# VITA-Group/CV_A-FAN

Measured on AMD Instinct MI355X. Metric: images/sec (whole node) A-FAN K=5 train step, ResNet-18/CIFAR-10, higher is better.
Workload: dtype bf16; 1 GPU; resnet18 CIFAR-10-shape A-FAN K=5 bf16, batch 256/GPU, perturb_idx 6, internal layout nhwc, 1xMI355X per rank (BASELINE configs[1]); global_batch=256, parallelism=dp1, hipgraph=True, in_launch_batchnorm=True

## Files before the change

### cv_a-fan_amd/_lib.py

```python
import ctypes as C
import os

_HERE = os.path.dirname(os.path.abspath(__file__))
LIB_PATH = os.environ.get("AFAN_HIP_LIB") or os.path.join(_HERE, "libafan_hip.so")

AFAN_F32, AFAN_BF16 = 0, 1
AFAN_NCHW, AFAN_NHWC = 0, 1
AFAN_ESHAPE = -3
_ERRORS = {-1: "AFAN_EDTYPE (unknown dtype code)", -2: "AFAN_EALIGN (misaligned pointer)",
           AFAN_ESHAPE: "AFAN_ESHAPE (bad sizes)", -4: "AFAN_ENULL (required pointer is NULL)",
           -5: "AFAN_ELAYOUT (unknown layout code)"}

_p, _i, _l, _f = C.c_void_p, C.c_int, C.c_int64, C.c_float

SIGNATURES = {
    "afan_version": (_i, []),
    "afan_arch": (C.c_char_p, []),
    "afan_pgd_step": (_i, [_p, _p, _i, _p, _p, _l, _f, _f, _i, _p]),
    "afan_tensor_clamp": (_i, [_p, _p, _p, _l, _p]),
    "afan_norms_workspace_floats": (_l, [_l, _l]),
    "afan_pgd_step_norms": (_i, [_p, _p, _i, _p, _p, _l, _l, _f, _f, _i, _p, _p, _p, _p]),
    "afan_perturb_norms": (_i, [_p, _p, _l, _l, _p, _p, _p, _p]),
    "afan_pgd_step_l2_workspace_floats": (_l, [_l, _l]),
    "afan_pgd_step_l2": (_i, [_p, _p, _i, _p, _p, _l, _l, _f, _f, _i, _p, _p, _p, _p]),
    "afan_axpy_noise": (_i, [_p, _p, _l, _f, _p, _p]),
    "afan_pgd_rand_start": (_i, [_p, _p, _p, _l, _l, _l, _l, _i, _f, _p, _p, _i, _p]),
    "afan_mix_feature": (_i, [_p, _p, _p, _l, _l, _l, _f, _i, _p]),
    "afan_mix_feature_nhwc": (_i, [_p, _p, _p, _l, _l, _l, _f, _i, _p]),
    "afan_lerp_points": (_i, [_p, _p, _p, _l, C.POINTER(_f), _i, _p]),
    "afan_lerp_mix": (_i, [_p, _p, _p, _l, _l, _l, C.POINTER(_f), _i, C.c_uint, _f, _i, _p]),
    "afan_sat_points_nhwc": (_i, [_p, _p, _p, _i, _l, _l, C.POINTER(_f), _i, C.c_uint, _f, _p]),
    "afan_head_max_classes": (_i, []),
    "afan_head_forward": (_i, [_p, _i, _l, _l, _l, _p, _p, _l, _p, _p, _p]),
    "afan_head_backward": (_i, [_p, _p, _p, _l, _l, _l, _l, _p, _i, _p, _p, _i, _p]),
    "afan_cross_entropy": (_i, [_p, _p, _l, _l, _p, _p, _p]),
    "afan_head_ce": (_i, [_p, _p, _i, _l, _l, _l, _p, _p, _p, _l, _p, _f, _p, _p, _p, _p, _p, _p, _p]),
    "afan_loss_mean": (_i, [_p, _l, _p, _p]),
    "afan_mix_w_workspace_floats": (_l, []),
    "afan_mix_w": (_i, [_p, _p, _p, _p, _i, _l, _p]),
    "afan_mix_w_backward": (_i, [_p, _i, _p, _p, _l, _p, _p, _i, _p]),
    "afan_bn_workspace_floats": (_l, [_l]),
    "afan_bn_acc_doubles": (_l, [_l]),
    "afan_bn_acc_supported": (_i, [_i, _l]),
    "afan_bn_set_running_updates": (_i, [_i]),
    "afan_bn_running_update": (_i, [_p, _l, C.c_double, _f, _f, _p, _p, _p, _p]),
    "afan_bn_running_update_batched": (_i, [_p, _p, _p, _p, _p, _p, _p, _p, _i, _p]),
    "afan_bn_train_forward_acc": (_i, [_p, _p, _p, _i, _l, _l, _l, _f, _f, _p, _p, _i, _p, _i, _p, _p, _p, _p, _i, _p]),
    "afan_bn_train_forward_acc_dual": (_i, [_p, _p, _p, _i, _l, _l, _l, _f, _f, _p, _p, _p, _p, _p, _p, _p, _f, _f, _p, _p, _p, _p,
                                            _p, _p, _p, _p]),
    "afan_bn_backward_acc": (_i, [_p, _p, _p, _p, _p, _i, _l, _l, _l, _p, _i, _p, _i, _p, _p, _i, _i, _p]),
    "afan_bn_backward_rows": (_i, [_p, _p, _p, _p, _p, _i, _l, _l, _l, _p, _p, _p, _p, _i, _p]),
    "afan_bn_backward_acc_rows": (_i, [_p, _p, _p, _p, _p, _i, _l, _l, _l, _p, _p, _p, _p, _i, _p]),
    "afan_bn_stats": (_i, [_p, _i, _i, _l, _l, _l, _f, _f, _p, _p, _p, _p, _p, _p]),
    "afan_bn_train_forward": (_i, [_p, _p, _p, _i, _i, _l, _l, _l, _f, _f, _p, _p, _i, _p, _p, _p, _p, _p, _p]),
    "afan_bn_apply": (_i, [_p, _p, _p, _i, _i, _l, _l, _l, _p, _p, _p, _p, _i, _p, _p]),
    "afan_bn_backward": (_i, [_p, _p, _p, _p, _p, _i, _i, _l, _l, _l, _p, _p, _p, _i, _p, _p, _p, _i, _p, _l, _p]),
    "afan_conv_supported": (_i, [_l, _l, _i, _i]),
    "afan_conv_fwd_nhwc_bf16": (_i, [_p, _p, _p, _l, _l, _l, _l, _l, _i, _i, _i, _p, _p, _p, _i, _p]),
    "afan_conv_fwd_affine_nhwc_bf16": (_i, [_p, _p, _p, _l, _l, _l, _l, _l, _i, _i, _i, _p, _p, _i, _i, _p]),
    "afan_conv_fwd_multi_nhwc_bf16": (_i, [_p, _p, _p, _i, _l, _l, _l, _l, _l, _p, _i, _p, _p, _p, _i, _p]),
    "afan_conv_fwd_tiles": (_l, [_l, _l, _l, _l, _l, _i, _i]),
    "afan_bn_train_forward_partials": (_i, [_p, _p, _p, _i, _l, _l, _l, _f, _f, _p, _p, _i, _p, _l, _p, _p, _p, _p, _p, _p]),
    "afan_conv_dgrad_nhwc_bf16": (_i, [_p, _p, _p, _l, _l, _l, _l, _l, _i, _i, _i, _p, _p, _p, _i, _p, _p, _p, _i, _p]),
    "afan_conv_dgrad_affine_nhwc_bf16": (_i, [_p, _p, _p, _l, _l, _l, _l, _l, _i, _i, _i, _p, _p, _i, _p]),
    "afan_conv_dgrad_dual_nhwc_bf16": (_i, [_p, _p, _p, _p, _l, _l, _l, _l, _l, _i, _i, _p, _p, _p, _p]),
    "afan_conv_dgrad_sc_nhwc_bf16": (_i, [_p, _p, _p, _p, _l, _l, _l, _l, _l, _p, _p, _i, _p, _p, _p, _p]),
    "afan_grid_barrier_bytes": (_i, []),
    "afan_grid_barrier_error_word": (_i, []),
    "afan_grid_barrier_shared_gpu": (_i, [_i]),
    "afan_conv_fwd_bn_nhwc_bf16": (_i, [_p, _p, _p, _p, _l, _l, _l, _l, _l, _i, _i, _p, _p, _p, _p, _f, _f, _p, _p, _p, _p, _p, _i, _p, _p, _p, _p,
                                        _f, _f, _p, _p, _p, _p, _p, _p]),
    "afan_conv_dgrad_bn_nhwc_bf16": (_i, [_p, _p, _p, _p, _l, _l, _l, _l, _l, _i, _i, _p, _p, _p, _i, _p, _p, _p, _p, _i, _p, _p, _p, _p, _p, _p,
                                          _p, _p]),
    "afan_conv_fwd_multi_bn_nhwc_bf16": (_i, [_p, _p, _p, _i, _l, _l, _l, _l, _l, _p, _i, _p, _p, _p, _p, _p, _p, _f, _f, _p, _p, _p, _p, _i, _p,
                                              _p]),
# ... 129 lines not shown
```

### cv_a-fan_amd/attack_algo.py

```python
import torch

from . import ops, pgd
from .resnet_s import _dense, _like_layout, fused_criterion, tail_end_kwargs

__all__ = ["PGD", "tensor_clamp", "linfball_proj", "l2ball_proj", "mix_feature", "get_sample_points", "last_norms"]

_last = {"l2": None, "linf": None}


def last_norms():
    return _last["l2"], _last["linf"]


def tensor_clamp(t, min, max, in_place=True):
    res = t if in_place else t.clone()
    ops.tensor_clamp_(res.data, min.contiguous(), max.contiguous())
    return res


def linfball_proj(center, radius, t, in_place=True):
    res = t if in_place else t.clone()
    zero = torch.zeros_like(res.data)
    ops.pgd_step_(res.data, zero, 0.0, x_clean=center.contiguous(), eps=float(radius), clip=True)
    return res


def l2ball_proj(center, radius, t, in_place=True):
    res = t if in_place else t.clone()
    data = res.data
    if _dense(data) is not data or data.dtype != torch.float32:
        raise ValueError("l2ball_proj: t must be a dense fp32 tensor (contiguous NCHW or channels_last)")
    ops.pgd_step_l2_(data, None, 0.0, x_clean=_like_layout(center.detach().float(), data), eps=float(radius), clip=True)
    return res


def PGD(x, loss_fn, y=None, model=None, steps=3, gamma=None, start_idx=1, layer_number=16, eps=(2 / 255),
        randinit=False, clip=False, with_norms=False, grad0=None, norm="linf", tail_end=False):
    if x.device.type != "cuda":
        raise ops.AfanLibraryError("PGD: x must live on the MI355X (no CPU path in this build)")
    pgd._check_norm(norm)
    lp = getattr(model, "compute_dtype", torch.float32) == torch.bfloat16
    if grad0 is not None and (randinit or steps < 1):
        raise ValueError("grad0 is the gradient at x: not with randinit, and only when there is a first step")
    x, x_adv, shadow = ops.pgd_init(_dense(x.detach()), want_shadow=lp and grad0 is None and not randinit)
    if lp and shadow is None:
        shadow = torch.empty_like(x, dtype=torch.bfloat16)
    if randinit and norm == "l2":
        u = _like_layout(torch.randn(x_adv.shape).to(x.device, non_blocking=True), x_adv)
        ops.pgd_step_l2_(x_adv, u, eps, clip=False, shadow=shadow)
    elif randinit:
        ops.axpy_noise_(x_adv, torch.rand(x_adv.shape).to(x.device, non_blocking=True), eps, shadow)
    l2 = linf = None
    loss_fn = fused_criterion(loss_fn, model)
    ce_kw = tail_end_kwargs(model, loss_fn, y, ops.one(x.device), want_value=False) if tail_end else {}
    for t in range(steps):
        if t == 0 and grad0 is not None:
            grad = grad0
        else:
            xin = (shadow if lp else x_adv).detach().requires_grad_(True)
            grad = pgd.input_gradient(lambda t: loss_fn(model(t, end_point=layer_number, start_point=start_idx, **ce_kw), y), xin)
        if with_norms and t == steps - 1:
            l2, linf = pgd.step(x_adv, grad, gamma, x, eps, clip, shadow, norms=True, norm=norm)
        else:
            pgd.step(x_adv, grad, gamma, x, eps, clip, shadow, norm=norm)
    if with_norms:
        if l2 is None:
            l2, linf = ops.perturb_norms(x_adv, x)
        _last["l2"], _last["linf"] = l2, linf
    x_adv.requires_grad_(True)
    if lp:
        x_adv._afan_shadow = shadow
    return x_adv


def mix_feature(clean_feature, adv_feature):
    return ops.mix_feature(_dense(clean_feature), _dense(adv_feature), 1e-5)


def sample_points_mixed(pointx, pointy, number, mix):
    px, py = _dense(pointx), _dense(pointy)
    if py.stride() != px.stride():
        py = _like_layout(py, px)
    return [pointx] + ops.lerp_mix(px, py, number, [bool(f) for f in mix])


def get_sample_points(pointx, pointy, number):
    px, py = _dense(pointx), _dense(pointy)
    if py.stride() != px.stride():
        py = _like_layout(py, px)
    inner = ops.lerp_points(px, py, number)
    return [pointx] + inner + [pointy]
```

### cv_a-fan_amd/ops.py

```python
import contextlib
import ctypes as C
import os
import threading

import torch

from . import _lib
from ._lib import AFAN_BF16, AFAN_ESHAPE, AFAN_F32, AFAN_NCHW, AFAN_NHWC, AfanLibraryError, check

_DT = {torch.float32: AFAN_F32, torch.bfloat16: AFAN_BF16}
_ws_cache = {}
_tls = threading.local()
class _Calls(dict):

    def __init__(self, conv, other):
        super().__init__(conv)
        self.other = dict(other)

    def __getitem__(self, k):
        return self.other[k] if k in self.other else super().__getitem__(k)

    def __contains__(self, k):
        return k in self.other or super().__contains__(k)

    def get(self, k, default=None):
        return self[k] if k in self else default

    def __setitem__(self, k, v):
        if k in self.other:
            self.other[k] = v
        else:
            super().__setitem__(k, v)


CALLS = _Calls({"conv_fwd": 0, "conv_dgrad": 0, "conv_wgrad": 0, "conv_general": 0, "vendor_conv": 0, "conv_bn_fused": 0},
               {"batch_crop_flip": 0, "seg_batch_aug": 0, "seg_batch_aug_jitter": 0, "seg_confusion": 0, "det_batch_resize": 0,
                "frozen_stem_image_grad": 0, "sat_points": 0, "head_ce": 0})


def _need(t, name, dtype=None):
    if not isinstance(t, torch.Tensor):
        raise TypeError(f"{name}: expected a torch.Tensor")
    if t.device.type != "cuda":
        raise AfanLibraryError(f"{name}: tensor is on '{t.device}'. The A-FAN kernels are MI355X-only; "
                               "there is no CPU path (the CPU restatement under oracle/ is test infrastructure).")
    if not _dense(t):
        raise ValueError(f"{name}: tensor must be dense (contiguous NCHW or channels_last)")
    if dtype is not None and t.dtype != dtype:
        raise TypeError(f"{name}: expected {dtype}, got {t.dtype}")
    return t


def _dense(t):
    return t.is_contiguous() or (t.dim() == 4 and t.is_contiguous(memory_format=torch.channels_last))


def layout_of(t):
    if t.dim() == 4 and not t.is_contiguous() and t.is_contiguous(memory_format=torch.channels_last):
        return AFAN_NHWC
    return AFAN_NCHW


def _strides_eq(a, b):
    return all(sa == sb for sa, sb, n in zip(a.stride(), b.stride(), a.shape) if n > 1)


def _same_layout(ref, *others):
    for o in others:
        if o is not None and ref.numel() > 0 and (o.shape != ref.shape or not _strides_eq(o, ref)):
            raise ValueError("operands must share shape and memory layout (strides): "
                             f"{tuple(ref.shape)}/{ref.stride()} vs {tuple(o.shape)}/{o.stride()}")


def _ptr(t):
    return None if t is None else C.c_void_p(t.data_ptr())


_raw_stream = torch._C._cuda_getCurrentRawStream


def _stream(t):
    return C.c_void_p(_raw_stream(t.device.index))


def _workspace(ref, nfloats, tag):
    key = (ref.device.index, _raw_stream(ref.device.index), tag)
    ws = _ws_cache.get(key)
    if ws is None or ws.numel() < nfloats:
        ws = torch.empty(max(int(nfloats), 1024), dtype=torch.float32, device=ref.device)
        _ws_cache[key] = ws
# ... 146 lines not shown
        return False


def pgd_step_(x_adv, grad, gamma, x_clean=None, eps=0.0, clip=False, shadow=None):
    lib = _lib.load()
    _need(x_adv, "x_adv", torch.float32)
    _need(grad, "grad")
    if grad.dtype not in _DT or grad.numel() != x_adv.numel():
        raise TypeError("grad must be fp32/bf16 with x_adv's number of elements")
    if clip:
        _need(x_clean, "x_clean", torch.float32)
        if x_clean.numel() != x_adv.numel():
            raise ValueError("x_clean must match x_adv")
    if shadow is not None:
        _need(shadow, "shadow", torch.bfloat16)
    _same_layout(x_adv, grad, x_clean if clip else None, shadow)
    check(lib.afan_pgd_step(_ptr(x_adv), _ptr(grad), _DT[grad.dtype], _ptr(x_clean) if clip else None,
                            _ptr(shadow), x_adv.numel(), float(gamma), float(eps), int(bool(clip)),
                            _stream(x_adv)), "afan_pgd_step")
    return x_adv


def tensor_clamp_(t, lo, hi):
    lib = _lib.load()
    _need(t, "t", torch.float32)
    _need(lo, "min", torch.float32)
    _need(hi, "max", torch.float32)
    if lo.numel() != t.numel() or hi.numel() != t.numel():
        raise ValueError("min/max must match t")
    check(lib.afan_tensor_clamp(_ptr(t), _ptr(lo), _ptr(hi), t.numel(), _stream(t)), "afan_tensor_clamp")
    return t


def pgd_step_norms_(x_adv, grad, gamma, x_clean, eps=0.0, clip=False, shadow=None):
    lib = _lib.load()
    _need(x_adv, "x_adv", torch.float32)
    _need(grad, "grad")
    _need(x_clean, "x_clean", torch.float32)
    if grad.dtype not in _DT or grad.numel() != x_adv.numel() or x_clean.numel() != x_adv.numel():
        raise TypeError("grad/x_clean must match x_adv")
    if shadow is not None:
        _need(shadow, "shadow", torch.bfloat16)
    _same_layout(x_adv, grad, x_clean, shadow)
    batch = x_adv.shape[0]
    per = x_adv.numel() // max(batch, 1)
    out = torch.empty(2, batch, dtype=torch.float32, device=x_adv.device)
    if batch == 0:
        return out[0], out[1]
    ws = _workspace(x_adv, lib.afan_norms_workspace_floats(batch, per), "norms")
    check(lib.afan_pgd_step_norms(_ptr(x_adv), _ptr(grad), _DT[grad.dtype], _ptr(x_clean), _ptr(shadow),
                                  batch, per, float(gamma), float(eps), int(bool(clip)), _ptr(ws),
                                  _ptr(out[0]), _ptr(out[1]), _stream(x_adv)), "afan_pgd_step_norms")
    return out[0], out[1]


def perturb_norms(x_adv, x_clean):
    lib = _lib.load()
    _need(x_adv, "x_adv", torch.float32)
    _need(x_clean, "x_clean", torch.float32)
    if x_clean.numel() != x_adv.numel():
        raise ValueError("x_clean must match x_adv")
    _same_layout(x_adv, x_clean)
    batch = x_adv.shape[0]
    per = x_adv.numel() // max(batch, 1)
    out = torch.empty(2, batch, dtype=torch.float32, device=x_adv.device)
    if batch == 0:
        return out[0], out[1]
    ws = _workspace(x_adv, lib.afan_norms_workspace_floats(batch, per), "norms")
    check(lib.afan_perturb_norms(_ptr(x_adv), _ptr(x_clean), batch, per, _ptr(ws), _ptr(out[0]),
                                 _ptr(out[1]), _stream(x_adv)), "afan_perturb_norms")
    return out[0], out[1]


def pgd_step_l2_(x_adv, grad, gamma, x_clean=None, eps=0.0, clip=False, shadow=None, want_norms=False):
    lib = _lib.load()
    _need(x_adv, "x_adv", torch.float32)
    if grad is not None:
        _need(grad, "grad")
        if grad.dtype not in _DT or grad.numel() != x_adv.numel():
            raise TypeError("grad must be fp32/bf16 with x_adv's number of elements")
    if clip or want_norms:
        _need(x_clean, "x_clean", torch.float32)
        if x_clean.numel() != x_adv.numel():
            raise ValueError("x_clean must match x_adv")
    else:
        x_clean = None
    if shadow is not None:
        _need(shadow, "shadow", torch.bfloat16)
    if x_adv.dim() < 1:
        raise ValueError("x_adv must have a batch dimension")
    _same_layout(x_adv, grad, x_clean, shadow)
    batch = x_adv.shape[0]
    per = x_adv.numel() // max(batch, 1)
    out = torch.empty(2, batch, dtype=torch.float32, device=x_adv.device) if want_norms else None
    if x_adv.numel():
        ws = _workspace(x_adv, lib.afan_pgd_step_l2_workspace_floats(batch, per), "l2_step")
        check(lib.afan_pgd_step_l2(_ptr(x_adv), _ptr(grad), _DT[grad.dtype] if grad is not None else 0, _ptr(x_clean), _ptr(shadow),
                                   batch, per, float(gamma), float(eps), int(bool(clip)), _ptr(ws),
                                   _ptr(out[0]) if want_norms else None, _ptr(out[1]) if want_norms else None, _stream(x_adv)),
              "afan_pgd_step_l2")
    return (x_adv, out[0], out[1]) if want_norms else x_adv


def axpy_noise_(x_adv, u, eps, shadow=None):
    lib = _lib.load()
    _need(x_adv, "x_adv", torch.float32)
# ... 1835 lines not shown
```

### cv_a-fan_amd/train_step.py

```python
import contextlib
import time

import torch
import torch.distributed as dist

from . import ops
from .arena import ArenaSGD, ParamArena
from .attack_algo import PGD, last_norms
from .grid_guard import GuardedTrainer


def warmup_lr(step, optimizer, warm_up_steps=200, max_lr=0.1):
    lr = step * max_lr / (warm_up_steps - 1)
    lr = min(lr, max_lr)
    for p in optimizer.param_groups:
        p["lr"] = lr
    return lr


class GradAllReducer:

    def __init__(self, arena, n_chunks=4, group=None):
        self.arena, self.group = arena, group
        self.world = dist.get_world_size(group) if dist.is_initialized() else 1
        self.chunks = _cut_chunks(arena, n_chunks)
        self.on_cuda = arena.grad.device.type == "cuda"
        self.stream = torch.cuda.Stream(device=arena.grad.device) if self.on_cuda else None
        self._pending = []
        self._hooks = []
        self._need, self._done = [], []
        self.diag = False
        self._diag_ranges, self._diag_wait, self._diag_host = [], None, []
        if self.world > 1:
            bounds = arena.offsets + [arena.numel]
            for ci, (start, end, first_param) in enumerate(self.chunks):
                members = [i for i in range(len(arena.params)) if start <= bounds[i] < end]
                self._need.append(len(members))
                self._done.append(0)
                for i in members:
                    self._hooks.append(arena.params[i].register_post_accumulate_grad_hook(self._make_hook(ci)))

    enabled = False

    def _make_hook(self, ci):
        def hook(_param):
            if not self.enabled:
                return
            self._done[ci] += 1
            if self._done[ci] == self._need[ci]:
                start, end, _ = self.chunks[ci]
                self._launch(start, end)
        return hook

    def begin(self, explicit=False):
        self.enabled = not explicit
        self._done = [0] * len(self.chunks)
        self._covered = []
        self._diag_ranges, self._diag_wait, self._diag_host = [], None, []
        ops.exchange_in_flight(False)

    def launch_params(self, p_lo, p_hi):
        if p_hi <= p_lo:
# ... 306 lines not shown
        self.perturb_idx = perturb_idx
        self.layer_number = layer_number if layer_number is not None else model.layer_number
        self.randinit, self.clip = randinit, clip
        self.arena = ParamArena(model)
        self.optimizer = ArenaSGD(self.arena, lr, momentum, weight_decay)
        self._init_exchange(model, group, allreduce_chunks, emulate_dp)
        import os
        self.ddp_overlap = self.reducer is not None and os.environ.get("AFAN_DDP_OVERLAP", "1") != "0"
        self.segmented = bool(segmented)
        self.batch_final = bool(batch_final)
        self._groupable_key, self._groupable = None, False
        self.share_head = bool(share_head)
        self.fold_clean = fold_clean if fold_clean is None else bool(fold_clean)
        self._fold_auto = {}
        self._init_schedule(bool(use_graph) and not randinit, graph_warmup)

    FOLD_MIN_ELEMS = 0

    def _fold_ok(self, inp):
        if self.fold_clean is False or not (self._share_head(inp) and self.steps >= 1 and not self.randinit):
            return False
        if self.fold_clean is None:
            key = tuple(inp.shape)
            if self._fold_auto.get(key) is None:
                self._fold_auto[key] = self._feature_elems(inp) >= self.FOLD_MIN_ELEMS
            return self._fold_auto[key]
        return True

    def _feature_elems(self, inp):
        m = self.model
        c, h, w = inp.shape[1], inp.shape[2], inp.shape[3]
        for mod in m.sequential_model[:self.perturb_idx]:
            c, h, w = _out_shape(mod, c, h, w)
        return inp.shape[0] * c * h * w

    def _forward_backward_folded(self, inp, target, overlap_allreduce):
        from . import ops, resnet_s
        m, idx, ln = self.model, self.perturb_idx, self.layer_number
        ops.acc_reset(inp.device)
        self.optimizer.zero_grad()
        crit = resnet_s.fused_criterion(self.criterion, m)
        half = ops.half(inp.device)
        with ops.bn_running_updates(2):
            fm_clean = m(inp, end_point=idx, start_point=0)
        xin = fm_clean.detach().requires_grad_(True)
        ce_kw = resnet_s.tail_end_kwargs(m, crit, target, half)
        with ops.record_bn_updates() as clean_bn:
            output_clean = m(xin, end_point=ln, start_point=idx, **ce_kw)
        loss_clean = crit(output_clean, target)
        with resnet_s.stash_wgrad():
            torch.autograd.backward(loss_clean, grad_tensors=half)
        g0 = xin.grad
        feature_map = fm_clean.detach()
        feature_map = feature_map.float() if feature_map.dtype != torch.float32 else feature_map
        feature_map_adv = PGD(feature_map, self.criterion, y=target, model=m, steps=self.steps,
                              gamma=(self.gamma / 255), start_idx=idx, layer_number=ln, eps=(self.eps / 255),
                              randinit=False, clip=self.clip, with_norms=True, grad0=g0, tail_end=True)
        l2, linf = last_norms()
        adv_in = getattr(feature_map_adv, "_afan_shadow", None)
        if adv_in is None:
            adv_in = feature_map_adv.detach()
        output_adv = m(adv_in, end_point=ln, start_point=idx, **ce_kw)
        loss_adv = crit(output_adv, target)
        torch.autograd.backward(loss_adv, grad_tensors=half)
        resnet_s.flush_wgrad(m)
        clean_bn.replay()
        if overlap_allreduce:
            self.reducer.begin()
        fm_clean.backward(g0)
        with torch.no_grad():
            loss = (loss_adv + loss_clean) / 2
            prec1 = (output_clean.argmax(dim=1) == target).float().sum() * (100.0 / target.shape[0])
        return {"loss": loss.detach(), "loss_adv": loss_adv.detach(), "loss_clean": loss_clean.detach(),
                "prec1": prec1, "l2": l2, "linf": linf, "x_adv": feature_map_adv.detach(),
                "feature_map": feature_map, "out_clean": output_clean.detach()}

    def _tail_segments(self):
        m, idx, ln = self.model, self.perturb_idx, self.layer_number
        cuts = [idx]
        for i in range(idx + 1, ln):
            mod = m.sequential_model[i]
            if getattr(mod, "_sc_kind", "identity") != "identity":
                cuts.append(i)
        cuts.append(ln)
        return [(cuts[k], cuts[k + 1]) for k in range(len(cuts) - 1)]

    def _param_range(self, a, b):
        pre = tuple(f"sequential_model.{i}." for i in range(a, b))
        idxs = [i for i, n in enumerate(self.arena.names) if n.startswith(pre)]
        return (idxs[0], idxs[-1] + 1) if idxs else (0, 0)

    def _phases(self, inp, target, out):
        from . import ops, resnet_s
        m, idx, ln = self.model, self.perturb_idx, self.layer_number
        segs = self._tail_segments()
        ops.acc_reset(inp.device)
        self.optimizer.zero_grad()
        crit = resnet_s.fused_criterion(self.criterion, m)
        half = ops.half(inp.device)

        ce_kw = resnet_s.tail_end_kwargs(m, crit, target, half)

        def run_segments(x0):
            ins, outs, h = [x0], [], x0
            for k, (a, b) in enumerate(segs):
                o = m(h, end_point=b, start_point=a, **(ce_kw if k + 1 == len(segs) else {}))
                outs.append(o)
                if k + 1 < len(segs):
                    h = o.detach().requires_grad_(True)
                    ins.append(h)
            return ins, outs

        with ops.bn_running_updates(2):
            fm_clean = m(inp, end_point=idx, start_point=0)
        xin = fm_clean.detach().requires_grad_(True)
        with ops.record_bn_updates() as clean_bn:
            c_ins, c_outs = run_segments(xin)
        loss_clean = crit(c_outs[-1], target)
        with resnet_s.stash_wgrad():
            torch.autograd.backward(loss_clean, grad_tensors=half)
            for k in range(len(segs) - 2, -1, -1):
                c_outs[k].backward(c_ins[k + 1].grad)
        g0 = xin.grad
        feature_map = fm_clean.detach()
        feature_map = feature_map.float() if feature_map.dtype != torch.float32 else feature_map
        feature_map_adv = PGD(feature_map, self.criterion, y=target, model=m, steps=self.steps,
                              gamma=(self.gamma / 255), start_idx=idx, layer_number=ln, eps=(self.eps / 255),
                              randinit=False, clip=self.clip, with_norms=True, grad0=g0, tail_end=True)
        l2, linf = last_norms()
        adv_in = getattr(feature_map_adv, "_afan_shadow", None)
        if adv_in is None:
            adv_in = feature_map_adv.detach()
        a_ins, a_outs = run_segments(adv_in)
        loss_adv = crit(a_outs[-1], target)
        torch.autograd.backward(loss_adv, grad_tensors=half)
        resnet_s.flush_wgrad(m.sequential_model[segs[-1][0]:segs[-1][1]])
        yield self._param_range(*segs[-1])
        with ops.grid_bn(self.reducer is None):
            for k in range(len(segs) - 2, -1, -1):
                a_outs[k].backward(a_ins[k + 1].grad)
                resnet_s.flush_wgrad(m.sequential_model[segs[k][0]:segs[k][1]])
                if k == 0:
                    clean_bn.replay()
                yield self._param_range(*segs[k])
            if len(segs) == 1:
                clean_bn.replay()
            fm_clean.backward(g0)
        with torch.no_grad():
            loss = (loss_adv + loss_clean) / 2
            prec1 = (c_outs[-1].argmax(dim=1) == target).float().sum() * (100.0 / target.shape[0])
        out.update({"loss": loss.detach(), "loss_adv": loss_adv.detach(), "loss_clean": loss_clean.detach(),
                    "prec1": prec1, "l2": l2, "linf": linf, "x_adv": feature_map_adv.detach(),
                    "feature_map": feature_map, "out_clean": c_outs[-1].detach()})
        yield self._param_range(0, idx)

    def _use_phases(self, inp):
        want = self.segmented or (self.ddp_overlap and self.reducer is not None)
        return bool(want and self._fold_ok(inp) and hasattr(self.model, "sequential_model"))

    def _piece_count(self):
        return len(self._tail_segments()) + 1

    def _forward_backward(self, inp, target, overlap_allreduce):
        if self._fold_ok(inp):
            return self._forward_backward_folded(inp, target, overlap_allreduce)
        m, idx, ln = self.model, self.perturb_idx, self.layer_number
        if inp.is_cuda:
            from . import ops
            ops.acc_reset(inp.device)
        fm_clean = None
        if self._share_head(inp):
            from . import ops
            with ops.bn_running_updates(2):
                fm_clean = m(inp, end_point=idx, start_point=0)
            feature_map = fm_clean.detach()
        else:
            with torch.no_grad():
                feature_map = m(inp, end_point=idx, start_point=0)
        feature_map = feature_map.float() if feature_map.dtype != torch.float32 else feature_map
        from . import resnet_s as _rsb
        with _rsb.bn_branch(m, "adv"):
            feature_map_adv = PGD(feature_map, self.criterion, y=target, model=m, steps=self.steps,
                                  gamma=(self.gamma / 255), start_idx=idx, layer_number=ln, eps=(self.eps / 255),
                                  randinit=self.randinit, clip=self.clip, with_norms=True)
        l2, linf = last_norms()
        adv_in = getattr(feature_map_adv, "_afan_shadow", None)
        if adv_in is None:
            adv_in = feature_map_adv.detach()
        if self.batch_final and self._tail_groupable(adv_in):
            from . import resnet_s
            if fm_clean is None:
                fm_clean = m(inp, end_point=idx, start_point=0)
            both = torch.cat([adv_in, fm_clean.to(adv_in.dtype)], dim=0)
            with resnet_s.bn_groups(2):
                out_both = m(both, end_point=ln, start_point=idx)
            nb = adv_in.shape[0]
            output_adv, output_clean = out_both[:nb], out_both[nb:]
        else:
            with _rsb.bn_branch(m, "adv"):
                output_adv = m(adv_in, end_point=ln, start_point=idx)
            output_clean = (m(fm_clean, end_point=ln, start_point=idx) if fm_clean is not None
                            else m(inp, end_point=ln, start_point=0))
        from . import resnet_s as _rs
        crit = _rs.fused_criterion(self.criterion, m)
        loss_adv = crit(output_adv.contiguous() if output_adv.dim() == 2 else output_adv, target)
        loss_clean = crit(output_clean.contiguous() if output_clean.dim() == 2 else output_clean, target)
        loss = (loss_adv + loss_clean) / 2
        self.optimizer.zero_grad()
        if overlap_allreduce:
            self.reducer.begin()
        from . import resnet_s
        if loss.is_cuda and loss.dtype == torch.float32 and loss.dim() == 0:
            from . import ops as _ops
            loss.backward(gradient=_ops.one(loss.device))
        else:
            loss.backward()
        with torch.no_grad():
            prec1 = (output_clean.argmax(dim=1) == target).float().sum() * (100.0 / target.shape[0])
        return {"loss": loss.detach(), "loss_adv": loss_adv.detach(), "loss_clean": loss_clean.detach(),
                "prec1": prec1, "l2": l2, "linf": linf, "x_adv": feature_map_adv.detach(),
                "feature_map": feature_map, "out_clean": output_clean.detach()}

    def _share_head(self, inp):
        m = self.model
        return bool(self.share_head and inp.is_cuda and self.perturb_idx > 0 and getattr(m, "channels_last", False)
                    and hasattr(m, "sequential_model") and m.training)

    def _tail_groupable(self, fea):
        from . import ops as _ops
        key = (tuple(fea.shape), fea.dtype, fea.is_contiguous(memory_format=torch.channels_last), _ops.BN_ACC)
        if self._groupable_key == key:
            return self._groupable
        from . import resnet_s
        from . import ops
        ok = (fea.is_cuda and fea.dim() == 4 and fea.dtype == torch.bfloat16 and key[2] and resnet_s._Flags.block_fusion
              and ops.BN_ACC)
        n, _, h, w = fea.shape if fea.dim() == 4 else (0, 0, 0, 0)
        if ok:
# ... 86 lines not shown
```

### include/afan_hip.h

```cpp
#ifndef AFAN_HIP_H
#define AFAN_HIP_H

#include <stdint.h>

#ifdef __cplusplus
extern "C" {
#endif

typedef void* afan_stream_t;

enum { AFAN_F32 = 0, AFAN_BF16 = 1 };

enum { AFAN_NCHW = 0, AFAN_NHWC = 1 };

enum {
    AFAN_OK = 0,
    AFAN_EDTYPE = -1,
    AFAN_EALIGN = -2,
    AFAN_ESHAPE = -3,
    AFAN_ENULL = -4,
    AFAN_ELAYOUT = -5
};

int afan_version(void);
const char* afan_arch(void);

int afan_pgd_step(float* x_adv, const void* grad, int grad_dtype, const float* x_clean,
                  uint16_t* shadow_bf16, int64_t n, float gamma, float eps, int clip,
                  afan_stream_t stream);

int afan_tensor_clamp(float* t, const float* lo, const float* hi, int64_t n, afan_stream_t stream);

int64_t afan_norms_workspace_floats(int64_t batch, int64_t per_sample);
int afan_pgd_step_norms(float* x_adv, const void* grad, int grad_dtype, const float* x_clean,
                        uint16_t* shadow_bf16, int64_t batch, int64_t per_sample, float gamma,
                        float eps, int clip, float* partial, float* l2_out, float* linf_out,
                        afan_stream_t stream);

int afan_perturb_norms(const float* x_adv, const float* x_clean, int64_t batch, int64_t per_sample,
                       float* partial, float* l2_out, float* linf_out, afan_stream_t stream);

int64_t afan_pgd_step_l2_workspace_floats(int64_t batch, int64_t per_sample);
int afan_pgd_step_l2(float* x_adv, const void* grad, int grad_dtype, const float* x_clean,
                     uint16_t* shadow_bf16, int64_t batch, int64_t per_sample,
                     float gamma, float eps, int clip, float* workspace,
                     float* gnorm_out, float* dnorm_out, afan_stream_t stream);

int afan_axpy_noise(float* x_adv, const float* u, int64_t n, float eps, uint16_t* shadow_bf16,
                    afan_stream_t stream);

int afan_pgd_rand_start(const float* x, float* x_adv, uint16_t* shadow_bf16, int64_t n, int64_t c, int64_t h, int64_t w,
                        int layout, float eps, uint64_t* state, uint64_t* used, int advance, afan_stream_t stream);

int afan_mix_feature(const void* clean, const void* adv, void* out, int64_t n, int64_t c, int64_t hw,
                     float eps, int dtype, afan_stream_t stream);
int afan_mix_feature_nhwc(const void* clean, const void* adv, void* out, int64_t n, int64_t c, int64_t hw, float eps,
                          int dtype, afan_stream_t stream);

int afan_lerp_points(const float* x, const float* y, float* out, int64_t n, const float* weights,
                     int n_interior, afan_stream_t stream);

int afan_lerp_mix(const float* clean, const float* adv, float* out, int64_t n, int64_t c, int64_t hw, const float* weights,
                  int n_points, unsigned mix_mask, float eps, int layout, afan_stream_t stream);

int afan_sat_points_nhwc(const float* clean, const float* adv, void* out, int out_dtype, int64_t pixels, int64_t c,
                         const float* weights, int n_points, unsigned mix_mask, float eps, afan_stream_t stream);

int64_t afan_mix_w_workspace_floats(void);
int afan_mix_w(const float* clean, const float* adv, const float* w, void* out, int out_dtype, int64_t n,
               afan_stream_t stream);
int afan_mix_w_backward(const void* grad_out, int grad_dtype, const float* clean, const float* adv, int64_t n,
                        float* workspace, float* dw, int accumulate, afan_stream_t stream);

int64_t afan_bn_workspace_floats(int64_t c);
int afan_bn_stats(const void* x, int dtype, int layout, int64_t n, int64_t c, int64_t hw, float eps,
                  float momentum, float* workspace, float* stats, float* running_mean, float* running_var,
                  int64_t* num_batches, afan_stream_t stream);

int afan_bn_train_forward(const void* x, const void* residual, void* y, int dtype, int layout, int64_t n,
                          int64_t c, int64_t hw, float eps, float momentum, const float* weight,
                          const float* bias, int relu, float* workspace, float* save_stats,
                          float* running_mean, float* running_var, int64_t* num_batches,
                          afan_stream_t stream);

int afan_bn_train_forward_partials(const void* x, const void* residual, void* y, int dtype, int64_t n, int64_t c,
                                   int64_t hw, float eps, float momentum, const float* weight, const float* bias,
                                   int relu, const float* partials, int64_t partials_g, const float* partials_shift,
                                   float* save_stats, float* running_mean, float* running_var,
                                   int64_t* num_batches, afan_stream_t stream);

int afan_bn_apply(const void* x, const void* residual, void* y, int dtype, int layout, int64_t n, int64_t c,
                  int64_t hw, const float* mean, const float* invstd, const float* weight, const float* bias,
                  int relu, float* workspace, afan_stream_t stream);
// ... 307 lines not shown
```

Baseline: 33740 images/sec.

## Replace fp32 PGD iterate with bf16 clean input plus packed 2-bit sign codes

When the feature map is bf16 and the attack is linf without random init, PGD no longer keeps an fp32 clean copy and an fp32 adversarial iterate. It keeps the bf16 clean input and a byte of 2-bit gradient-sign codes per element, and rebuilds the iterate each step by replaying the recorded signs. The last step writes the fp32 adversarial tensor, an fp32 clean copy and the per-sample norms in one fused kernel. This cuts the upfront fp32 cast and the per-step fp32 read/write traffic, at the cost of extra replay arithmetic per element and a hard limit of five steps.

```diff
diff --git a/cv_a-fan_amd/_lib.py b/cv_a-fan_amd/_lib.py
--- a/cv_a-fan_amd/_lib.py
+++ b/cv_a-fan_amd/_lib.py
@@ -21,6 +21,8 @@
     "afan_norms_workspace_floats": (_l, [_l, _l]),
     "afan_pgd_step_norms": (_i, [_p, _p, _i, _p, _p, _l, _l, _f, _f, _i, _p, _p, _p, _p]),
     "afan_perturb_norms": (_i, [_p, _p, _l, _l, _p, _p, _p, _p]),
+    "afan_pgd_packed_step": (_i, [_p, _p, _i, _p, _i, _l, _f, _f, _i, _p, _p]),
+    "afan_pgd_packed_last": (_i, [_p, _p, _i, _p, _i, _l, _l, _f, _f, _i, _p, _p, _p, _p, _p, _p, _p]),
     "afan_pgd_step_l2_workspace_floats": (_l, [_l, _l]),
     "afan_pgd_step_l2": (_i, [_p, _p, _i, _p, _p, _l, _l, _f, _f, _i, _p, _p, _p, _p]),
     "afan_axpy_noise": (_i, [_p, _p, _l, _f, _p, _p]),
diff --git a/cv_a-fan_amd/attack_algo.py b/cv_a-fan_amd/attack_algo.py
--- a/cv_a-fan_amd/attack_algo.py
+++ b/cv_a-fan_amd/attack_algo.py
@@ -1,3 +1,5 @@
+import os
+
 import torch
 
 from . import ops, pgd
@@ -6,6 +8,13 @@
 __all__ = ["PGD", "tensor_clamp", "linfball_proj", "l2ball_proj", "mix_feature", "get_sample_points", "last_norms"]
 
 _last = {"l2": None, "linf": None}
+_PGD_PACKED = os.environ.get("AFAN_PGD_PACKED", "1") != "0"
+
+
+def pgd_packed_ok(x, model, steps, norm="linf", randinit=False):
+    return bool(_PGD_PACKED and isinstance(x, torch.Tensor) and x.device.type == "cuda" and x.dtype == torch.bfloat16
+                and getattr(model, "compute_dtype", torch.float32) == torch.bfloat16 and norm == "linf" and not randinit
+                and 1 <= steps <= ops.PGD_PACKED_MAX_STEPS)
 
 
 def last_norms():
@@ -42,6 +51,9 @@
     lp = getattr(model, "compute_dtype", torch.float32) == torch.bfloat16
     if grad0 is not None and (randinit or steps < 1):
         raise ValueError("grad0 is the gradient at x: not with randinit, and only when there is a first step")
+    if pgd_packed_ok(x, model, steps, norm, randinit):
+        return _pgd_packed(_dense(x.detach()), loss_fn, y, model, steps, gamma, start_idx, layer_number, eps, clip, with_norms, grad0,
+                           tail_end)
     x, x_adv, shadow = ops.pgd_init(_dense(x.detach()), want_shadow=lp and grad0 is None and not randinit)
     if lp and shadow is None:
         shadow = torch.empty_like(x, dtype=torch.bfloat16)
@@ -73,6 +85,34 @@
     return x_adv
 
 
+def _pgd_packed(x, loss_fn, y, model, steps, gamma, start_idx, layer_number, eps, clip, with_norms, grad0, tail_end):
+    if eps is None:
+        if clip:
+            raise ValueError("clip=True needs an eps")
+        eps = 0.0
+    codes = torch.empty_like(x, dtype=torch.uint8) if steps > 1 else None
+    shadow = torch.empty_like(x)
+    loss_fn = fused_criterion(loss_fn, model)
+    ce_kw = tail_end_kwargs(model, loss_fn, y, ops.one(x.device), want_value=False) if tail_end else {}
+    for t in range(steps):
+        if t == 0 and grad0 is not None:
+            grad = grad0
+        else:
+            xin = (x if t == 0 else shadow).detach().requires_grad_(True)
+            grad = pgd.input_gradient(lambda t: loss_fn(model(t, end_point=layer_number, start_point=start_idx, **ce_kw), y), xin)
+        grad = _like_layout(grad.detach(), x)
+        if t < steps - 1:
+            ops.pgd_packed_step_(x, grad, codes, t, gamma, eps, clip, shadow)
+        else:
+            x_adv, x32, l2, linf = ops.pgd_packed_last(x, grad, codes, t, gamma, eps, clip, shadow, want_x32=True, norms=with_norms)
+    if with_norms:
+        _last["l2"], _last["linf"] = l2, linf
+    x_adv.requires_grad_(True)
+    x_adv._afan_shadow = shadow
+    x_adv._afan_clean32 = x32
+    return x_adv
+
+
 def mix_feature(clean_feature, adv_feature):
     return ops.mix_feature(_dense(clean_feature), _dense(adv_feature), 1e-5)
 
diff --git a/cv_a-fan_amd/csrc/afan_pgd_packed.hip b/cv_a-fan_amd/csrc/afan_pgd_packed.hip
--- /dev/null
+++ b/cv_a-fan_amd/csrc/afan_pgd_packed.hip
@@ -0,0 +1,313 @@
+#include "afan_common.h"
+
+using namespace afan;
+
+namespace {
+
+constexpr int BLOCK = 256;
+constexpr int NORM_CHUNK = 4096;
+constexpr int TRIPS = NORM_CHUNK / (BLOCK * 4);
+constexpr int MAX_CODES = 4;
+
+__device__ __forceinline__ float sign_of(float g) {
+    return (g != g) ? g : (float)((g > 0.f) - (g < 0.f));
+}
+
+__device__ __forceinline__ uint32_t code_of(float g) { return (g != g) ? 3u : (g > 0.f) ? 1u : (g < 0.f) ? 2u : 0u; }
+__device__ __forceinline__ float sign_from(uint32_t c) { return c == 0u ? 0.f : c == 1u ? 1.f : c == 2u ? -1.f : __builtin_nanf(""); }
+
+template <bool CLIP>
+__device__ __forceinline__ float step_signed(float xa, float s, float xc, float gamma, float eps) {
+    float d = gamma * s;
+    float t = xa + d;
+    if (CLIP) {
+        float lo = xc - eps;
+        float hi = xc + eps;
+        if (t < lo) t = lo;
+        if (t > hi) t = hi;
+    }
+    return t;
+}
+
+template <bool CLIP>
+__device__ __forceinline__ float step_one(float xa, float g, float xc, float gamma, float eps) {
+    return step_signed<CLIP>(xa, sign_of(g), xc, gamma, eps);
+}
+
+template <bool CLIP, int T>
+__device__ __forceinline__ float replay(float xc, uint32_t byte, float gamma, float eps) {
+    float xa = xc;
+#pragma unroll
+    for (int s = 0; s < T; ++s) xa = step_signed<CLIP>(xa, sign_from((byte >> (2 * s)) & 3u), xc, gamma, eps);
+    return xa;
+}
+
+template <int T>
+__device__ __forceinline__ uint32_t with_code(uint32_t byte, float g) {
+    return (byte & ((1u << (2 * T)) - 1u)) | (code_of(g) << (2 * T));
+}
+
+template <typename G> struct GradVec4;
+template <> struct GradVec4<float> {
+    __device__ static __forceinline__ void ld(const float* p, float (&g)[4]) { Elt<float>::ldv(p, g); }
+};
+template <> struct GradVec4<uint16_t> {
+    __device__ static __forceinline__ void ld(const uint16_t* p, float (&g)[4]) {
+        u16x4 t = *reinterpret_cast<const u16x4*>(p);
+#pragma unroll
+        for (int i = 0; i < 4; ++i) g[i] = bf2f(t[i]);
+    }
+};
+
+template <typename G, bool CLIP, bool VEC, int T>
+__global__ __launch_bounds__(BLOCK) void pgd_packed_step_kernel(const uint16_t* __restrict__ x0, const G* __restrict__ grad,
+                                                                uint8_t* __restrict__ codes, uint16_t* __restrict__ shadow,
+                                                                int64_t n, float gamma, float eps) {
+    const int64_t tid = (int64_t)blockIdx.x * BLOCK + threadIdx.x;
+    const int64_t nthreads = (int64_t)gridDim.x * BLOCK;
+    int64_t done = 0;
+    if (VEC) {
+        const int64_t nvec = n >> 3;
+        for (int64_t v = tid; v < nvec; v += nthreads) {
+            const int64_t i = v << 3;
+            float xc[8], g[8], xa[8];
+            Elt<uint16_t>::ldv(x0 + i, xc);
+            if constexpr (sizeof(G) == 4) {
+                float a[4], b[4];
+                Elt<float>::ldv((const float*)grad + i, a);
+                Elt<float>::ldv((const float*)grad + i + 4, b);
+#pragma unroll
+                for (int k = 0; k < 4; ++k) { g[k] = a[k]; g[4 + k] = b[k]; }
+            } else {
+                Elt<uint16_t>::ldv((const uint16_t*)grad + i, g);
+            }
+            uint32_t c[2] = {0u, 0u}, o[2] = {0u, 0u};
+            if (T > 0) {
+                const uint2 cc = *reinterpret_cast<const uint2*>(codes + i);
+                c[0] = cc.x;
+                c[1] = cc.y;
+            }
+#pragma unroll
+            for (int k = 0; k < 8; ++k) {
+                const uint32_t byte = (c[k >> 2] >> (8 * (k & 3))) & 0xffu;
+                xa[k] = step_one<CLIP>(replay<CLIP, T>(xc[k], byte, gamma, eps), g[k], xc[k], gamma, eps);
+                o[k >> 2] |= with_code<T>(byte, g[k]) << (8 * (k & 3));
+            }
+            *reinterpret_cast<uint2*>(codes + i) = make_uint2(o[0], o[1]);
+            Elt<uint16_t>::stv(shadow + i, xa);
+        }
+        done = nvec << 3;
+    }
+    for (int64_t i = done + tid; i < n; i += nthreads) {
+        const float xc = bf2f(x0[i]), g = Elt<G>::ld(grad + i);
+        const uint32_t byte = T > 0 ? (uint32_t)codes[i] : 0u;
+        const float t = step_one<CLIP>(replay<CLIP, T>(xc, byte, gamma, eps), g, xc, gamma, eps);
+        codes[i] = (uint8_t)with_code<T>(byte, g);
+        shadow[i] = f2bf(t);
+    }
+}
+
+__device__ __forceinline__ void block_reduce_store(float ss, float mx, float* __restrict__ partial, int64_t slot) {
+    __shared__ float s_ss[BLOCK / AFAN_WAVE];
+    __shared__ float s_mx[BLOCK / AFAN_WAVE];
+    ss = wave_sum(ss);
+    const float nanflag = wave_max((mx != mx) ? 1.f : 0.f);
+    mx = wave_max((mx != mx) ? 0.f : mx);
+    if (nanflag > 0.f) mx = __builtin_nanf("");
+    const int lane = threadIdx.x & 63, w = threadIdx.x >> 6;
+    if (lane == 0) {
+        s_ss[w] = ss;
+        s_mx[w] = mx;
+    }
+    __syncthreads();
+    if (threadIdx.x == 0) {
+        float a = 0.f, b = 0.f;
+#pragma unroll
+        for (int k = 0; k < BLOCK / AFAN_WAVE; ++k) {
+            a += s_ss[k];
+            b = (b != b || s_mx[k] != s_mx[k]) ? __builtin_nanf("") : fmaxf(b, s_mx[k]);
+        }
+        partial[2 * slot] = a;
+        partial[2 * slot + 1] = b;
+    }
+}
+
+__device__ __forceinline__ float absmax_nan(float m, float d) {
+    float a = fabsf(d);
+    return (a != a || m != m) ? __builtin_nanf("") : fmaxf(m, a);
+}
+
+template <typename G, bool CLIP, bool VEC, int T>
+__global__ __launch_bounds__(BLOCK) void pgd_packed_last_kernel(const uint16_t* __restrict__ x0, const G* __restrict__ grad,
+                                                                const uint8_t* __restrict__ codes, float* __restrict__ x32,
+                                                                float* __restrict__ x_adv, uint16_t* __restrict__ shadow,
+                                                                int64_t per_sample, float gamma, float eps,
+                                                                float* __restrict__ partial) {
+    const int64_t b = blockIdx.y;
+    const int64_t base = b * per_sample;
+    const int64_t lo = (int64_t)blockIdx.x * NORM_CHUNK;
+    const int64_t hi = (lo + NORM_CHUNK < per_sample) ? lo + NORM_CHUNK : per_sample;
+    float ss = 0.f, mx = 0.f;
+    if (VEC) {
+        float xc[TRIPS][4], g[TRIPS][4];
+        uint32_t c[TRIPS];
+#pragma unroll
+        for (int r = 0; r < TRIPS; ++r) {
+            const int64_t j = lo + (int64_t)threadIdx.x * 4 + (int64_t)r * (BLOCK * 4);
+            c[r] = 0u;
+            if (j < hi) {
+                const int64_t i = base + j;
+                GradVec4<uint16_t>::ld(x0 + i, xc[r]);
+                GradVec4<G>::ld(grad + i, g[r]);
+                if (T > 0) c[r] = *reinterpret_cast<const uint32_t*>(codes + i);
+            }
+        }
+#pragma unroll
+        for (int r = 0; r < TRIPS; ++r) {
+            const int64_t j = lo + (int64_t)threadIdx.x * 4 + (int64_t)r * (BLOCK * 4);
+            if (j < hi) {
+                const int64_t i = base + j;
+                float xa[4];
+#pragma unroll
+                for (int k = 0; k < 4; ++k)
+                    xa[k] = step_one<CLIP>(replay<CLIP, T>(xc[r][k], (c[r] >> (8 * k)) & 0xffu, gamma, eps), g[r][k], xc[r][k], gamma, eps);
+                Elt<float>::stv(x_adv + i, xa);
+                if (x32) Elt<float>::stv(x32 + i, xc[r]);
+                if (shadow) {
+                    u16x4 s;
+#pragma unroll
+                    for (int k = 0; k < 4; ++k) s[k] = f2bf(xa[k]);
+                    *reinterpret_cast<u16x4*>(shadow + i) = s;
+                }
+#pragma unroll
+                for (int k = 0; k < 4; ++k) {
+                    float d = xa[k] - xc[r][k];
+                    ss += d * d;
+                    mx = absmax_nan(mx, d);
+                }
+            }
+        }
+    } else {
+        for (int64_t j = lo + threadIdx.x; j < hi; j += BLOCK) {
+            const int64_t i = base + j;
+            const float xc = bf2f(x0[i]);
+            const uint32_t byte = T > 0 ? (uint32_t)codes[i] : 0u;
+            const float xa = step_one<CLIP>(replay<CLIP, T>(xc, byte, gamma, eps), Elt<G>::ld(grad + i), xc, gamma, eps);
+            x_adv[i] = xa;
+            if (x32) x32[i] = xc;
+            if (shadow) shadow[i] = f2bf(xa);
+            float d = xa - xc;
+            ss += d * d;
+            mx = absmax_nan(mx, d);
+        }
+    }
+    if (partial) block_reduce_store(ss, mx, partial, b * gridDim.x + blockIdx.x);
+}
+
+__global__ __launch_bounds__(AFAN_WAVE) void pgd_packed_finalize_kernel(const float* __restrict__ partial, int slices,
+                                                                        float* __restrict__ l2, float* __restrict__ linf) {
+    const int64_t b = blockIdx.x;
+    float ss = 0.f, mx = 0.f;
+    for (int s = threadIdx.x; s < slices; s += AFAN_WAVE) {
+        ss += partial[2 * (b * slices + s)];
+        float m = partial[2 * (b * slices + s) + 1];
+        mx = (m != m || mx != mx) ? __builtin_nanf("") : fmaxf(mx, m);
+    }
+    ss = wave_sum(ss);
+    float isn = (mx != mx) ? 1.f : 0.f;
+    isn = wave_max(isn);
+    mx = wave_max((mx != mx) ? 0.f : mx);
+    if (threadIdx.x == 0) {
+        l2[b] = sqrtf(ss);
+        linf[b] = (isn > 0.f) ? __builtin_nanf("") : mx;
+    }
+}
+
+#define AFAN_EACH_T(X, TMAX)      \
+    switch (t) {                  \
+        case 0: X(0) break;       \
+        case 1: X(1) break;       \
+        case 2: X(2) break;       \
+        case 3: X(3) break;       \
+        default:                  \
+            if (TMAX > 3) { X(TMAX) } \
+            break;                \
+    }
+
+template <typename G, bool CLIP>
+int launch_step(const uint16_t* x0, const void* grad, uint8_t* codes, int t, int64_t n, float gamma, float eps, uint16_t* shadow,
+                hipStream_t st) {
+    const bool vec = aligned(x0, 16) && aligned(grad, 16) && aligned(codes, 8) && aligned(shadow, 16);
+    const int grid = grid_for(vec ? (n + 7) / 8 : n, BLOCK);
+    AFAN_PROF("pgd_step_kernel", n * (2.0 + sizeof(G) + (t > 0 ? 1 : 0) + 1 + 2), st);
+#define AFAN_STEP(T_)                                                                                                            \
+    if (vec) pgd_packed_step_kernel<G, CLIP, true, T_><<<grid, BLOCK, 0, st>>>(x0, (const G*)grad, codes, shadow, n, gamma, eps); \
+    else pgd_packed_step_kernel<G, CLIP, false, T_><<<grid, BLOCK, 0, st>>>(x0, (const G*)grad, codes, shadow, n, gamma, eps);
+    AFAN_EACH_T(AFAN_STEP, 3)
+#undef AFAN_STEP
+    AFAN_LAUNCH_CHECK();
+    return AFAN_OK;
+}
+
+template <typename G, bool CLIP>
+int launch_last(const uint16_t* x0, const void* grad, const uint8_t* codes, int t, int64_t batch, int64_t per_sample, float gamma,
+                float eps, float* x32, float* x_adv, uint16_t* shadow, float* partial, float* l2, float* linf, hipStream_t st) {
+    const bool vec = (per_sample % 4 == 0) && aligned(x0, 8) && aligned(grad, 4 * sizeof(G)) && (t == 0 || aligned(codes, 4)) &&
+                     aligned(x_adv, 16) && (!x32 || aligned(x32, 16)) && (!shadow || aligned(shadow, 8));
+    const int slices = (int)((per_sample + NORM_CHUNK - 1) / NORM_CHUNK);
+    dim3 grid(slices, (unsigned)batch);
+    {
+        const double elts = (double)batch * (double)per_sample;
+        AFAN_PROF("pgd_step_norms_kernel", elts * (2.0 + sizeof(G) + (t > 0 ? 1 : 0) + 4 + (x32 ? 4 : 0) + (shadow ? 2 : 0)), st);
+#define AFAN_LAST(T_)                                                                                                         \
+    if (vec) pgd_packed_last_kernel<G, CLIP, true, T_><<<grid, BLOCK, 0, st>>>(x0, (const G*)grad, codes, x32, x_adv, shadow, \
+                                                                               per_sample, gamma, eps, partial);              \
+    else pgd_packed_last_kernel<G, CLIP, false, T_><<<grid, BLOCK, 0, st>>>(x0, (const G*)grad, codes, x32, x_adv, shadow,    \
+                                                                            per_sample, gamma, eps, partial);
+        AFAN_EACH_T(AFAN_LAST, 4)
+#undef AFAN_LAST
+        AFAN_LAUNCH_CHECK();
+    }
+    if (partial) {
+        AFAN_PROF("norms_finalize_kernel", 8.0 * batch * slices, st);
+        pgd_packed_finalize_kernel<<<(unsigned)batch, AFAN_WAVE, 0, st>>>(partial, slices, l2, linf);
+        AFAN_LAUNCH_CHECK();
+    }
+    return AFAN_OK;
+}
+
+}
+
+extern "C" {
+
+int afan_pgd_packed_step(const uint16_t* x0, const void* grad, int grad_dtype, uint8_t* codes, int t, int64_t n, float gamma,
+                         float eps, int clip, uint16_t* shadow, afan_stream_t stream) {
+    if (n < 0 || t < 0 || t >= MAX_CODES) return AFAN_ESHAPE;
+    if (n == 0) return AFAN_OK;
+    if (!x0 || !grad || !codes || !shadow) return AFAN_ENULL;
+    if (grad_dtype != AFAN_F32 && grad_dtype != AFAN_BF16) return AFAN_EDTYPE;
+    hipStream_t st = (hipStream_t)stream;
+    if (grad_dtype == AFAN_F32)
+        return clip ? launch_step<float, true>(x0, grad, codes, t, n, gamma, eps, shadow, st)
+                    : launch_step<float, false>(x0, grad, codes, t, n, gamma, eps, shadow, st);
+    return clip ? launch_step<uint16_t, true>(x0, grad, codes, t, n, gamma, eps, shadow, st)
+                : launch_step<uint16_t, false>(x0, grad, codes, t, n, gamma, eps, shadow, st);
+}
+
+int afan_pgd_packed_last(const uint16_t* x0, const void* grad, int grad_dtype, const uint8_t* codes, int t, int64_t batch,
+                         int64_t per_sample, float gamma, float eps, int clip, float* x32, float* x_adv, uint16_t* shadow,
+                         float* workspace, float* l2, float* linf, afan_stream_t stream) {
+    if (batch < 0 || per_sample <= 0 || batch > 65535 || t < 0 || t > MAX_CODES) return AFAN_ESHAPE;
+    if (batch == 0) return AFAN_OK;
+    if (!x0 || !grad || !x_adv || (t > 0 && !codes) || (l2 && (!linf || !workspace))) return AFAN_ENULL;
+    if (grad_dtype != AFAN_F32 && grad_dtype != AFAN_BF16) return AFAN_EDTYPE;
+    hipStream_t st = (hipStream_t)stream;
+    float* partial = l2 ? workspace : nullptr;
+    if (grad_dtype == AFAN_F32)
+        return clip ? launch_last<float, true>(x0, grad, codes, t, batch, per_sample, gamma, eps, x32, x_adv, shadow, partial, l2, linf, st)
+                    : launch_last<float, false>(x0, grad, codes, t, batch, per_sample, gamma, eps, x32, x_adv, shadow, partial, l2, linf, st);
+    return clip ? launch_last<uint16_t, true>(x0, grad, codes, t, batch, per_sample, gamma, eps, x32, x_adv, shadow, partial, l2, linf, st)
+                : launch_last<uint16_t, false>(x0, grad, codes, t, batch, per_sample, gamma, eps, x32, x_adv, shadow, partial, l2, linf, st);
+}
+
+}
diff --git a/cv_a-fan_amd/ops.py b/cv_a-fan_amd/ops.py
--- a/cv_a-fan_amd/ops.py
+++ b/cv_a-fan_amd/ops.py
@@ -35,7 +35,7 @@
 
 CALLS = _Calls({"conv_fwd": 0, "conv_dgrad": 0, "conv_wgrad": 0, "conv_general": 0, "vendor_conv": 0, "conv_bn_fused": 0},
                {"batch_crop_flip": 0, "seg_batch_aug": 0, "seg_batch_aug_jitter": 0, "seg_confusion": 0, "det_batch_resize": 0,
-                "frozen_stem_image_grad": 0, "sat_points": 0, "head_ce": 0})
+                "frozen_stem_image_grad": 0, "sat_points": 0, "head_ce": 0, "pgd_packed": 0})
 
 
 def _need(t, name, dtype=None):
@@ -288,6 +288,49 @@
                                   batch, per, float(gamma), float(eps), int(bool(clip)), _ptr(ws),
                                   _ptr(out[0]), _ptr(out[1]), _stream(x_adv)), "afan_pgd_step_norms")
     return out[0], out[1]
+
+
+PGD_PACKED_MAX_STEPS = 5
+
+
+def _packed_args(x0, grad, codes, t, shadow):
+    _need(x0, "x0", torch.bfloat16)
+    _need(grad, "grad")
+    if grad.dtype not in _DT or grad.numel() != x0.numel():
+        raise TypeError("grad must be fp32/bf16 with x0's number of elements")
+    if codes is not None:
+        _need(codes, "codes", torch.uint8)
+    if shadow is not None:
+        _need(shadow, "shadow", torch.bfloat16)
+    _same_layout(x0, grad, codes, shadow)
+
+
+def pgd_packed_step_(x0, grad, codes, t, gamma, eps=0.0, clip=False, shadow=None):
+    lib = _lib.load()
+    _packed_args(x0, grad, codes, t, shadow)
+    if codes is None or shadow is None:
+        raise ValueError("pgd_packed_step_ writes codes and shadow: both are required")
+    check(lib.afan_pgd_packed_step(_ptr(x0), _ptr(grad), _DT[grad.dtype], _ptr(codes), int(t), x0.numel(), float(gamma), float(eps),
+                                   int(bool(clip)), _ptr(shadow), _stream(x0)), "afan_pgd_packed_step")
+    CALLS["pgd_packed"] += 1
+    return shadow
+
+
+def pgd_packed_last(x0, grad, codes, t, gamma, eps=0.0, clip=False, shadow=None, want_x32=True, norms=True):
+    lib = _lib.load()
+    _packed_args(x0, grad, codes, t, shadow)
+    batch = x0.shape[0] if x0.dim() else 1
+    per = x0.numel() // max(batch, 1)
+    x_adv = torch.empty_like(x0, dtype=torch.float32)
+    x32 = torch.empty_like(x0, dtype=torch.float32) if want_x32 else None
+    out = torch.empty(2, batch, dtype=torch.float32, device=x0.device) if norms else None
+    if x0.numel():
+        ws = _workspace(x0, lib.afan_norms_workspace_floats(batch, per), "norms") if norms else None
+        check(lib.afan_pgd_packed_last(_ptr(x0), _ptr(grad), _DT[grad.dtype], _ptr(codes), int(t), batch, per, float(gamma), float(eps),
+                                       int(bool(clip)), _ptr(x32), _ptr(x_adv), _ptr(shadow), _ptr(ws), _ptr(out[0]) if norms else None,
+                                       _ptr(out[1]) if norms else None, _stream(x0)), "afan_pgd_packed_last")
+        CALLS["pgd_packed"] += 1
+    return x_adv, x32, (out[0] if norms else None), (out[1] if norms else None)
 
 
 def perturb_norms(x_adv, x_clean):
diff --git a/cv_a-fan_amd/train_step.py b/cv_a-fan_amd/train_step.py
--- a/cv_a-fan_amd/train_step.py
+++ b/cv_a-fan_amd/train_step.py
@@ -6,8 +6,14 @@
 
 from . import ops
 from .arena import ArenaSGD, ParamArena
-from .attack_algo import PGD, last_norms
+from .attack_algo import PGD, last_norms, pgd_packed_ok
 from .grid_guard import GuardedTrainer
+
+
+def _pgd_input(feature_map, model, steps, randinit=False):
+    if pgd_packed_ok(feature_map, model, steps, randinit=randinit):
+        return feature_map
+    return feature_map.float() if feature_map.dtype != torch.float32 else feature_map
 
 
 def warmup_lr(step, optimizer, warm_up_steps=200, max_lr=0.1):
@@ -420,11 +426,12 @@
             torch.autograd.backward(loss_clean, grad_tensors=half)
         g0 = xin.grad
         feature_map = fm_clean.detach()
-        feature_map = feature_map.float() if feature_map.dtype != torch.float32 else feature_map
+        feature_map = _pgd_input(feature_map, m, self.steps)
         feature_map_adv = PGD(feature_map, self.criterion, y=target, model=m, steps=self.steps,
                               gamma=(self.gamma / 255), start_idx=idx, layer_number=ln, eps=(self.eps / 255),
                               randinit=False, clip=self.clip, with_norms=True, grad0=g0, tail_end=True)
         l2, linf = last_norms()
+        feature_map = getattr(feature_map_adv, "_afan_clean32", feature_map)
         adv_in = getattr(feature_map_adv, "_afan_shadow", None)
         if adv_in is None:
             adv_in = feature_map_adv.detach()
@@ -491,11 +498,12 @@
                 c_outs[k].backward(c_ins[k + 1].grad)
         g0 = xin.grad
         feature_map = fm_clean.detach()
-        feature_map = feature_map.float() if feature_map.dtype != torch.float32 else feature_map
+        feature_map = _pgd_input(feature_map, m, self.steps)
         feature_map_adv = PGD(feature_map, self.criterion, y=target, model=m, steps=self.steps,
                               gamma=(self.gamma / 255), start_idx=idx, layer_number=ln, eps=(self.eps / 255),
                               randinit=False, clip=self.clip, with_norms=True, grad0=g0, tail_end=True)
         l2, linf = last_norms()
+        feature_map = getattr(feature_map_adv, "_afan_clean32", feature_map)
         adv_in = getattr(feature_map_adv, "_afan_shadow", None)
         if adv_in is None:
             adv_in = feature_map_adv.detach()
@@ -545,13 +553,14 @@
         else:
             with torch.no_grad():
                 feature_map = m(inp, end_point=idx, start_point=0)
-        feature_map = feature_map.float() if feature_map.dtype != torch.float32 else feature_map
+        feature_map = _pgd_input(feature_map, m, self.steps, self.randinit)
         from . import resnet_s as _rsb
         with _rsb.bn_branch(m, "adv"):
             feature_map_adv = PGD(feature_map, self.criterion, y=target, model=m, steps=self.steps,
                                   gamma=(self.gamma / 255), start_idx=idx, layer_number=ln, eps=(self.eps / 255),
                                   randinit=self.randinit, clip=self.clip, with_norms=True)
         l2, linf = last_norms()
+        feature_map = getattr(feature_map_adv, "_afan_clean32", feature_map)
         adv_in = getattr(feature_map_adv, "_afan_shadow", None)
         if adv_in is None:
             adv_in = feature_map_adv.detach()
diff --git a/include/afan_hip.h b/include/afan_hip.h
--- a/include/afan_hip.h
+++ b/include/afan_hip.h
@@ -39,6 +39,12 @@
 
 int afan_perturb_norms(const float* x_adv, const float* x_clean, int64_t batch, int64_t per_sample,
                        float* partial, float* l2_out, float* linf_out, afan_stream_t stream);
+
+int afan_pgd_packed_step(const uint16_t* x0, const void* grad, int grad_dtype, uint8_t* codes, int t, int64_t n, float gamma,
+                         float eps, int clip, uint16_t* shadow, afan_stream_t stream);
+int afan_pgd_packed_last(const uint16_t* x0, const void* grad, int grad_dtype, const uint8_t* codes, int t, int64_t batch,
+                         int64_t per_sample, float gamma, float eps, int clip, float* x32, float* x_adv, uint16_t* shadow,
+                         float* workspace, float* l2, float* linf, afan_stream_t stream);
 
 int64_t afan_pgd_step_l2_workspace_floats(int64_t batch, int64_t per_sample);
 int afan_pgd_step_l2(float* x_adv, const void* grad, int grad_dtype, const float* x_clean,
```

Measured after the change: 34130 images/sec, median of 6. 1.1% higher.
